# jsnchon/acai-omr

Hardware: AMD Instinct MI355X
Metric: LMX tokens/sec (greedy decode, KV cache) (higher is better)
Workload: dtype bf16; 1 GPU; vitomr_greedy_decode batch 8/GPU of 512x2048 images (4096 patches), decode steps 6..136; batch_per_gpu=8, memory_len=4096, decoder=12 x d1024 h16 mlp4096, V=227, hipgraph=True, split_merge=in-launch

## Files before the change

### acai_omr_amd/_lib.py

```python
import ctypes
import os
import subprocess
from ctypes import POINTER, Structure, c_char_p, c_float, c_int, c_int32, c_int64, c_uint32, c_void_p, c_size_t

CSRC = os.path.join(os.path.dirname(os.path.abspath(__file__)), "csrc")
LIB_PATH = os.environ.get("ACAI_OMR_LIB") or os.path.join(CSRC, "libacai_omr_hip.so")
SOURCES = ["gemm.hip", "elementwise.hip", "attn_varlen.hip", "attn_fwd64.hip", "attn_fwd64w.hip", "attn_bwd.hip", "attn_bwd64w.hip", "attn_bwd1p.hip", "train.hip", "grpo.hip", "seqdist.hip", "decode.hip", "resize.hip"]

ACAI_F32, ACAI_BF16, ACAI_FP8_E4M3 = 0, 1, 2
GEMM_GELU, GEMM_ROUND_BF16 = 1, 2
DEC_CROSS_FP8 = 256


class AcaiDecLayer(Structure):
    _fields_ = [(n, c_void_p) for n in (
        "self_in_w", "self_in_b", "self_out_w", "self_out_b", "cross_q_w", "cross_q_b", "cross_out_w", "cross_out_b",
        "lin1_w", "lin1_b", "lin2_w", "lin2_b", "n1_w", "n1_b", "n2_w", "n2_b", "n3_w", "n3_b",
        "k_self", "v_self", "k_cross", "v_cross", "k_cross_scale", "v_cross_scale")]


class AcaiAdamWTensor(Structure):
    _fields_ = [("p", c_void_p), ("g", c_void_p), ("m", c_void_p), ("v", c_void_p), ("n", c_int64), ("group", c_int32), ("pad_", c_int32),
                ("bias_c1", c_float), ("bias_c2_sqrt", c_float)]

# ... 50 lines not shown
    "acai_attn_varlen_bwd_ws": (c_int, [c_void_p, c_int, c_void_p, c_int, c_void_p, c_int, c_void_p, c_int, c_void_p, c_int, c_void_p, c_int,
                                        c_void_p, c_int, c_void_p, c_int, c_void_p, c_void_p, c_void_p, c_void_p, c_int, c_int, c_int, c_int, c_int,
                                        c_int, c_int, c_int, c_int, c_float, c_uint32, c_int, c_void_p, c_size_t, c_void_p]),
    "acai_attn_varlen_bwd_workspace_bytes": (c_size_t, [c_int, c_int, c_int, c_int, c_int, c_int, c_int, c_int, c_int, c_float, c_int]),
    "acai_dropout_add": (c_int, [c_void_p, c_void_p, c_void_p, c_int, c_int, c_float, c_uint32, c_int, c_int, c_void_p]),
    "acai_layernorm_bwd": (c_int, [c_void_p, c_void_p, c_void_p, c_float, c_void_p, c_void_p, c_void_p, c_void_p, c_void_p, c_void_p, c_int, c_int, c_void_p]),
    "acai_gelu_fwd": (c_int, [c_void_p, c_void_p, c_int64, c_int, c_void_p]),
    "acai_gelu_bwd": (c_int, [c_void_p, c_void_p, c_void_p, c_int64, c_int, c_void_p]),
    "acai_adamw_step": (c_int, [c_void_p, c_void_p, c_void_p, c_void_p, c_int, c_int, c_float, c_void_p]),
    "acai_cast_weights": (c_int, [c_void_p, c_int, c_int, c_void_p]),
    "acai_gemm_dw": (c_int, [c_void_p, c_int, c_void_p, c_int, c_void_p, c_int, c_void_p, c_int, c_int, c_int, c_int, c_void_p]),
    "acai_colsum": (c_int, [c_void_p, c_int, c_void_p, c_int, c_int, c_int, c_void_p]),
    "acai_scatter_add_rows": (c_int, [c_void_p, c_void_p, c_void_p, c_int, c_int, c_int, c_void_p]),
    "acai_mae_loss": (c_int, [c_void_p, c_void_p, c_void_p, c_float, c_void_p, c_void_p, c_int, c_int, c_void_p]),
    "acai_ce_loss": (c_int, [c_void_p, c_int, c_void_p, c_int, c_float, c_float, c_void_p, c_void_p, c_int, c_int, c_void_p]),
    "acai_grpo_objective_fwd": (c_int, [c_void_p, c_int, c_void_p, c_int, c_void_p, c_int, c_void_p, c_void_p, c_int, c_int, c_int, c_float, c_float,
                                        c_int, c_float, c_void_p, c_void_p, c_void_p, c_void_p]),
    "acai_grpo_objective_bwd": (c_int, [c_void_p, c_int, c_void_p, c_int, c_void_p, c_void_p, c_void_p, c_void_p, c_int, c_int, c_int, c_int, c_float,
                                        c_void_p, c_void_p]),
    "acai_edit_distance": (c_int, [c_void_p, c_int, c_void_p, c_void_p, c_int, c_void_p, c_int, c_int, c_void_p, c_void_p]),
    "acai_debug_stamps": (c_int, [c_void_p, c_int]),
    "acai_debug_lds_dma_oob": (c_int, [c_void_p, c_int, c_void_p, c_void_p]),
    "acai_pe_interp_fwd": (c_int, [c_void_p, c_int, c_int, c_int, c_void_p, c_int, c_int, c_void_p]),
    "acai_pe_interp_bwd": (c_int, [c_void_p, c_int, c_int, c_int, c_void_p, c_int, c_int, c_void_p]),
    "acai_cast_f32_bf16": (c_int, [c_void_p, c_void_p, c_int64, c_void_p]),
    "acai_skinny_gemm": (c_int, [c_void_p, c_int, c_void_p, c_int, c_void_p, c_void_p, c_int, c_void_p, c_int, c_int, c_int, c_int,
                                 c_int, c_int, c_void_p]),
    "acai_skinny_gemm_ex": (c_int, [c_void_p, c_int, c_int, c_void_p, c_int, c_void_p, c_void_p, c_int, c_void_p, c_int, c_int, c_int, c_int,
                                    c_int, c_int, c_int, c_void_p, c_void_p, c_float, c_void_p, c_void_p, c_void_p, c_void_p, c_void_p]),
    "acai_decode_attn": (c_int, [c_void_p, c_int, c_void_p, c_void_p, c_void_p, c_void_p, c_void_p, c_void_p, c_int, c_int, c_int,
                                 c_int, c_int, c_int, c_int, c_int, c_int, c_void_p, c_void_p]),
    "acai_decode_attn_fp8": (c_int, [c_void_p, c_int, c_void_p, c_void_p, c_void_p, c_void_p, c_void_p, c_void_p, c_void_p, c_void_p, c_int,
                                     c_int, c_int, c_int, c_int, c_int, c_int, c_int, c_void_p, c_void_p]),
    "acai_cross_kv_quantize_fp8": (c_int, [c_void_p, c_void_p, c_void_p, c_void_p, c_void_p, c_void_p, c_int64, c_int64, c_int, c_void_p]),
    "acai_decode_embed": (c_int, [POINTER(AcaiDecoder), c_void_p]),
    "acai_decode_step": (c_int, [POINTER(AcaiDecoder), c_void_p]),
    "acai_decode_sample_step": (c_int, [POINTER(AcaiDecoder), c_void_p, c_int, c_float, c_void_p]),
    "acai_decode_beam_step": (c_int, [POINTER(AcaiDecoder), POINTER(AcaiBeam), c_void_p]),
    "acai_decode_slot_step": (c_int, [POINTER(AcaiDecoder), POINTER(AcaiSlots), c_void_p]),
    "acai_decode_slot_sample_step": (c_int, [POINTER(AcaiDecoder), POINTER(AcaiSlots), c_void_p, c_int, c_void_p, c_int, c_float,
                                             c_void_p]),
    "acai_decode_slot_arm": (c_int, [POINTER(AcaiDecoder), POINTER(AcaiSlots), c_void_p, c_int, c_void_p]),
    "acai_decode_logits": (c_int, [POINTER(AcaiDecoder), c_void_p, c_int, c_void_p]),
    "acai_decode_hidden": (c_int, [POINTER(AcaiDecoder), c_void_p, c_void_p]),
    "acai_decode_merge_in_launch": (c_int, [c_int, c_int]),
    "acai_graph_begin": (c_int, [c_void_p]),
    "acai_graph_end": (c_int, [c_void_p, POINTER(c_void_p)]),
    "acai_graph_launch": (c_int, [c_void_p, c_void_p]),
    "acai_graph_destroy": (c_int, [c_void_p]),
}

_lib = None


def build(force=False, verbose=False):
    from concurrent.futures import ThreadPoolExecutor
    srcs = [os.path.join(CSRC, s) for s in SOURCES if os.path.exists(os.path.join(CSRC, s))]
    hdrs = sorted(os.path.join(CSRC, f) for f in os.listdir(CSRC) if f.endswith(".h")) + [os.path.join(os.path.dirname(CSRC), "..", "include", "acai_omr_hip.h")]
    hipcc = "hipcc" if subprocess.run(["which", "hipcc"], capture_output=True).returncode == 0 else "/opt/rocm/bin/hipcc"
    flags = ["-O3", "--offload-arch=gfx950", "-std=c++17", "-fPIC", "-Wno-unused-value"]
    per_file = {"attn_varlen.hip": ["-fno-slp-vectorize"], "attn_fwd64.hip": ["-fno-slp-vectorize"],
                "attn_fwd64w.hip": ["-fno-slp-vectorize", "-mllvm", "-amdgpu-mfma-vgpr-form"], "attn_bwd.hip": ["-fno-slp-vectorize"],
                "attn_bwd64w.hip": ["-fno-slp-vectorize", "-mllvm", "-amdgpu-mfma-vgpr-form"],
                "attn_bwd1p.hip": ["-fno-slp-vectorize", "-mllvm", "-amdgpu-mfma-vgpr-form"]}
    objdir = os.path.join(CSRC, "build")
    os.makedirs(objdir, exist_ok=True)
# ... 74 lines not shown
```

### acai_omr_amd/csrc/decode.hip

```cpp
#include <stdlib.h>

#include "common.h"

#include <mutex>
#include <unordered_map>

namespace {

constexpr int SK_KC = 1024;
constexpr int SK_BC = 8;

struct SkinnyArgs {
    const float *x;
    const void *W;
    const float *bias;
    const float *residual;
    float *y;
    int ldx, ldw, ldr, ldy, B, N, K, flags;
    void *k_cache, *v_cache;
    const int32_t *step;
    int E, H, dh, dhp, Tmax;
    const float *ln_w, *ln_b;
    float ln_eps;
    float *stats_out;
// ... 656 lines not shown
    const void *kc, *vc;
    const int64_t *seq_off;
    const int32_t *seq_len;
    const int32_t *step;
    float *partial;
    int ldq, H, dh, dhp, Tmax, chunk, nsplit;
    float scale_log2e;
    float *out;
    int ldo, round_out;
    unsigned *tickets;
    union {
        const int32_t *anc;
        const int32_t *slot_first;
    };
    int anc_pitch;
    long long anc_bstride;
    const float *k_scale, *v_scale;
};

struct fp8e4m3_t {
    uint8_t bits;
};

template <typename TC, int LPK, bool RAGGED, int U = 2, bool ANC = false, bool SLOT = false>
__global__ __launch_bounds__(256) void decode_attn_kernel(DAttnArgs a) {
    static_assert(!(ANC && RAGGED), "the ancestor table indexes the self-attention cache");
    static_assert(!(SLOT && (RAGGED || ANC)), "the ring indexes the self-attention cache of the row itself");
    constexpr bool F8 = sizeof(TC) == 1;
    static_assert(!F8 || RAGGED, "FP8 storage is the cross K/V's only");
    constexpr int EPC = 16 / sizeof(TC), KPW = 64 / LPK;
    __shared__ float red[4][2 + 64];
    const int tid = threadIdx.x, lane = tid & 63, wave = tid >> 6;
    const int kq = lane % LPK, kg = lane / LPK;
    const int split = blockIdx.x, h = blockIdx.y, b = blockIdx.z;
    int len, hstride;
    size_t base;
    if constexpr (RAGGED) {
        len = a.seq_len[b];
        hstride = len * a.dhp;
        base = (size_t)a.seq_off[b] + (size_t)h * hstride;
    } else if constexpr (ANC) {
        len = a.step[1] + 1;
        hstride = a.Tmax * a.dhp;
        base = (size_t)h * hstride;
    } else if constexpr (SLOT) {
        len = a.seq_len[b];
        hstride = a.Tmax * a.dhp;
        base = ((size_t)b * a.H + h) * hstride;
    } else {
        len = a.step[1] + 1;
        hstride = a.Tmax * a.dhp;
        base = ((size_t)b * a.H + h) * hstride;
    }
    float *part = a.partial + (((size_t)b * a.H + h) * a.nsplit + split) * (a.dhp + 2);
    const int c0 = split * a.chunk, c1 = min(len, c0 + a.chunk);
    const bool fused_merge = a.tickets && a.out && a.nsplit > 1;
    if (c0 >= len) {
        if (tid < a.dhp + 2) {
            if (fused_merge) __hip_atomic_store(part + tid, tid == 0 ? -1.0e30f : 0.f, __ATOMIC_RELAXED, __HIP_MEMORY_SCOPE_AGENT);
            else part[tid] = tid == 0 ? -1.0e30f : 0.f;
        }
        if (!fused_merge) return;
        asm volatile("s_waitcnt vmcnt(0)" ::: "memory");
    }
    const TC *Kp = reinterpret_cast<const TC *>(a.kc) + base;
    const TC *Vp = reinterpret_cast<const TC *>(a.vc) + base;
    [[maybe_unused]] const float *Ks = nullptr, *Vs = nullptr;
    if constexpr (F8) {
        const size_t row0 = base >> __builtin_ctz(a.dhp);
        Ks = a.k_scale + row0;
        Vs = a.v_scale + row0;
    }
    [[maybe_unused]] int32_t *anc_s = nullptr;
    if constexpr (ANC) {
        extern __shared__ int32_t anc_dyn[];
        anc_s = anc_dyn;
        const int32_t *ar = a.anc + (size_t)(a.step[0] & 1) * a.anc_bstride + (size_t)b * a.anc_pitch;
        for (int p = c0 + tid; p < c1; p += 256) anc_s[p - c0] = ar[p];
        __syncthreads();
    }
    [[maybe_unused]] int ring0 = 0;
    if constexpr (SLOT) ring0 = a.slot_first[b];
    auto key_off = [&](int key) -> size_t {
        if constexpr (ANC) return (size_t)anc_s[key - c0] * a.H * hstride + (size_t)key * a.dhp;
        else if constexpr (SLOT) {
            const int p = ring0 + key;
            return (size_t)(p >= a.Tmax ? p - a.Tmax : p) * a.dhp;
        } else return (size_t)key * a.dhp;
    };
// ... 96 lines not shown
    }
    float mw = m;
#pragma unroll
    for (int o = LPK; o < 64; o <<= 1) mw = fmaxf(mw, __shfl_xor(mw, o));
    const float f = fast_exp2(m - mw);
    l *= f;
#pragma unroll
    for (int e = 0; e < EPC; ++e) acc[e] *= f;
#pragma unroll
    for (int o = LPK; o < 64; o <<= 1) {
        l += __shfl_xor(l, o);
#pragma unroll
        for (int e = 0; e < EPC; ++e) acc[e] += __shfl_xor(acc[e], o);
    }
    if (kg == 0) {
        if (kq == 0) {
            red[wave][0] = mw;
            red[wave][1] = l;
        }
#pragma unroll
        for (int e = 0; e < EPC; ++e) red[wave][2 + kq * EPC + e] = acc[e];
    }
    __syncthreads();
    if (wave != 0) return;
    const int d = lane;
    const float M = fmaxf(fmaxf(red[0][0], red[1][0]), fmaxf(red[2][0], red[3][0]));
    float v = 0.f, lsum = 0.f;
#pragma unroll
    for (int w = 0; w < 4; ++w) {
        const float f = fast_exp2(red[w][0] - M);
        v += red[w][2 + d] * f;
        lsum += red[w][1] * f;
    }
    if (a.nsplit == 1 && a.out) {
        if (d < a.dh) {
            float o = v / lsum;
            if (a.round_out) o = round_bf16(o);
            a.out[(size_t)b * a.ldo + h * a.dh + d] = o;
        }
        return;
    }
    if (c0 < len && d < a.dhp) {
        if (fused_merge) {
            __hip_atomic_store(part + 2 + d, v, __ATOMIC_RELAXED, __HIP_MEMORY_SCOPE_AGENT);
            if (d == 0) {
                __hip_atomic_store(part, M, __ATOMIC_RELAXED, __HIP_MEMORY_SCOPE_AGENT);
                __hip_atomic_store(part + 1, lsum, __ATOMIC_RELAXED, __HIP_MEMORY_SCOPE_AGENT);
            }
        } else {
            part[2 + d] = v;
            if (d == 0) {
                part[0] = M;
                part[1] = lsum;
            }
        }
    }
    if (!fused_merge) return;
    asm volatile("s_waitcnt vmcnt(0)" ::: "memory");
    int last = 0;
    if (lane == 0) {
        unsigned *cnt = a.tickets + (size_t)b * a.H + h;
        const unsigned t = __hip_atomic_fetch_add(cnt, 1u, __ATOMIC_RELAXED, __HIP_MEMORY_SCOPE_AGENT);
        last = t == (unsigned)(a.nsplit - 1);
        if (last) __hip_atomic_store(cnt, 0u, __ATOMIC_RELAXED, __HIP_MEMORY_SCOPE_AGENT);
    }
    last = __builtin_amdgcn_readfirstlane(last);
    if (!last || d >= a.dhp) return;
    float *p = a.partial + ((size_t)b * a.H + h) * a.nsplit * (a.dhp + 2);
    auto ld = [&](int i) { return __hip_atomic_load(p + i, __ATOMIC_RELAXED, __HIP_MEMORY_SCOPE_AGENT); };
    float Mm = -1.0e30f, lm = 0.f, om = 0.f;
    for (int s0 = 0; s0 < a.nsplit; s0 += 8) {
        float pm[8], pl[8], po[8];
#pragma unroll
        for (int u = 0; u < 8; ++u) {
            const bool in = s0 + u < a.nsplit;
            const int pb = (in ? s0 + u : s0) * (a.dhp + 2);
            pm[u] = in ? ld(pb) : -1.0e30f;
            pl[u] = in ? ld(pb + 1) : 0.f;
            po[u] = in ? ld(pb + 2 + d) : 0.f;
        }
        float Mc = Mm;
#pragma unroll
        for (int u = 0; u < 8; ++u) Mc = fmaxf(Mc, pm[u]);
        const float resc = fast_exp2(Mm - Mc);
        lm *= resc;
        om *= resc;
        Mm = Mc;
#pragma unroll
        for (int u = 0; u < 8; ++u) {
            const float w = fast_exp2(pm[u] - Mm);
            lm += pl[u] * w;
            om += po[u] * w;
        }
    }
    if (d < a.dh) {
        float o = om / lm;
        if (a.round_out) o = round_bf16(o);
        a.out[(size_t)b * a.ldo + h * a.dh + d] = o;
    }
}

__global__ __launch_bounds__(256) void decode_attn_gmfma_kernel(DAttnArgs a, int group, int gtiles) {
    typedef bf16_t TC;
    typedef TileLayout<2, 64> TL;
    constexpr int GT = 16, KT = 32, DHP = 64;
    __shared__ __attribute__((aligned(16))) unsigned char vlds[4][KT * DHP * 2];
    __shared__ float red[4][GT][2 + 64];
    const int tid = threadIdx.x, lane = tid & 63, wave = tid >> 6;
// ... 622 lines not shown
        }
        if (t + 1 < a.Tmax)
            for (int i = lane * 4; i < a.E; i += 256) {
                const float4 ev = *reinterpret_cast<const float4 *>(a.emb + (size_t)tk * a.E + i), pv = *reinterpret_cast<const float4 *>(a.pos + (size_t)(t + 1) * a.E + i);
                *reinterpret_cast<float4 *>(a.x + (size_t)row * a.E + i) = make_float4(ev.x + pv.x, ev.y + pv.y, ev.z + pv.z, ev.w + pv.w);
            }
    }
}

inline int launch_dattn_group(const DAttnArgs &a, int B, int group, hipStream_t st) {
    const int gtm = cdiv(group, 16);
    hipLaunchKernelGGL(decode_attn_gmfma_kernel, dim3(a.nsplit, a.H, (B / group) * gtm), dim3(256), 0, st, a, group, gtm);
    ACAI_LAUNCH_CHECK("decode_attn_gmfma");
    return 0;
}

inline int launch_dattn_fp8(const DAttnArgs &a, int B, hipStream_t st) {
    if (!a.seq_off || !a.k_scale || !a.v_scale) return acai_set_err(-1, "decode_attn: the FP8 cache form needs ragged offsets and K / V scales");
    dim3 grid(a.nsplit, a.H, B);
    switch (a.dhp) {
        case 16: hipLaunchKernelGGL((decode_attn_kernel<fp8e4m3_t, 1, true>), grid, dim3(256), 0, st, a); break;
        case 32: hipLaunchKernelGGL((decode_attn_kernel<fp8e4m3_t, 2, true>), grid, dim3(256), 0, st, a); break;
        case 64: hipLaunchKernelGGL((decode_attn_kernel<fp8e4m3_t, 4, true>), grid, dim3(256), 0, st, a); break;
        default: return acai_set_err(-1, "decode_attn: FP8 cache dhp=%d unsupported (16, 32 or 64)", a.dhp);
    }
    ACAI_LAUNCH_CHECK("decode_attn_fp8");
    return 0;
}

template <typename TC>
int launch_dattn(const DAttnArgs &a, int B, hipStream_t st) {
    const int lpk = a.dhp * (int)sizeof(TC) / 16;
    static const int dattn_u = getenv("ACAI_DATTN_U") ? atoi(getenv("ACAI_DATTN_U")) : 2;
    dim3 grid(a.nsplit, a.H, B);
#define ACAI_DA(L)                                                                                        \
    case L:                                                                                               \
        if (a.seq_off && L == 8 && dattn_u == 4) hipLaunchKernelGGL((decode_attn_kernel<TC, 8, true, 4>), grid, dim3(256), 0, st, a);  \
        else if (a.seq_off && L == 8 && dattn_u == 3) hipLaunchKernelGGL((decode_attn_kernel<TC, 8, true, 3>), grid, dim3(256), 0, st, a);  \
        else if (a.seq_off) hipLaunchKernelGGL((decode_attn_kernel<TC, L, true>), grid, dim3(256), 0, st, a);  \
        else if (a.seq_len) hipLaunchKernelGGL((decode_attn_kernel<TC, L, false, 2, false, true>), grid, dim3(256), 0, st, a);             \
        else if (a.anc) hipLaunchKernelGGL((decode_attn_kernel<TC, L, false, 2, true>), grid, dim3(256), sizeof(int32_t) * a.chunk, st, a); \
        else hipLaunchKernelGGL((decode_attn_kernel<TC, L, false>), grid, dim3(256), 0, st, a);           \
        break;
    switch (lpk) {
        ACAI_DA(1) ACAI_DA(2) ACAI_DA(4) ACAI_DA(8) ACAI_DA(16)
        default: return acai_set_err(-1, "decode_attn: dhp=%d unsupported", a.dhp);
    }
#undef ACAI_DA
    ACAI_LAUNCH_CHECK("decode_attn");
    return 0;
}

template <typename TC>
bool dattn_merge_validated(int dhp) {
    static int cached[5] = {-1, -1, -1, -1, -1};
    static const int force = getenv("ACAI_DATTN_MERGE") ? atoi(getenv("ACAI_DATTN_MERGE")) : -1;
    if (force >= 0) return force != 0;
    const int lpk = dhp * (int)sizeof(TC) / 16;
    int idx = lpk == 1 ? 0 : lpk == 2 ? 1 : lpk == 4 ? 2 : lpk == 8 ? 3 : lpk == 16 ? 4 : -1;
    if (idx < 0) return false;
    if (cached[idx] < 0) {
        auto occ = [](int L, int &n) -> hipError_t {
            switch (L) {
#define ACAI_OCC(LL) case LL: return hipOccupancyMaxActiveBlocksPerMultiprocessor(&n, reinterpret_cast<const void *>(&decode_attn_kernel<TC, LL, true>), 256, 0);
                ACAI_OCC(1) ACAI_OCC(2) ACAI_OCC(4) ACAI_OCC(8) ACAI_OCC(16)
#undef ACAI_OCC
            }
// ... 93 lines not shown
            s.k_cache = kvl->k_self; s.v_cache = kvl->v_self; s.step = d->step;
            s.E = E; s.H = H; s.dh = d->dh; s.dhp = d->dhp; s.Tmax = d->Tmax;
        }
        return launch_skinny<TW>(s, st);
    };
    auto unembed = [&](const float *x, const float *lnw, const float *lnb, float eps, const float *ln2w, const float *ln2b) -> int {
        return skinny(x, E, d->unembed_w, d->unembed_b, nullptr, d->logits, d->V, d->V, E, rnd, nullptr, lnw, lnb, nullptr, nullptr, nullptr,
                      nullptr, eps, ln2w, ln2b);
    };
    const bool cross_f8 = (d->flags & ACAI_DEC_CROSS_FP8) != 0;
    auto attend = [&](const float *q, int ldq, const void *kc, const void *vc, bool cross, const AcaiDecLayer *ly = nullptr) -> int {
        DAttnArgs a{};
        a.q = q; a.kc = kc; a.vc = vc; a.ldq = ldq; a.H = H; a.dh = d->dh; a.dhp = d->dhp; a.Tmax = d->Tmax;
        a.partial = d->partial; a.scale_log2e = sc;
        if (cross && cross_f8) {
            a.seq_off = d->cross_off; a.seq_len = d->cross_len; a.chunk = d->cross_chunk; a.nsplit = d->cross_nsplit;
            a.dhp = d->dhp < 16 ? 16 : d->dhp;
            a.k_scale = ly->k_cross_scale; a.v_scale = ly->v_cross_scale;
            if (a.nsplit == 1 || (d->tickets && dattn_merge_validated_fp8(a.dhp))) {
                a.out = d->attn; a.ldo = E; a.round_out = rnd ? 1 : 0;
                if (a.nsplit > 1) a.tickets = d->tickets;
                return launch_dattn_fp8(a, B, st);
            }
            int r = launch_dattn_fp8(a, B, st);
            if (r) return r;
            hipLaunchKernelGGL(attn_combine_kernel, dim3(H, B), dim3(64), 0, st, d->partial, d->attn, E, H, d->dh, a.dhp, a.nsplit, rnd ? 1 : 0);
            ACAI_LAUNCH_CHECK("attn_combine");
            return 0;
        }
        if (cross) {
            a.seq_off = d->cross_off; a.seq_len = d->cross_len; a.chunk = d->cross_chunk; a.nsplit = d->cross_nsplit;
        } else {
            a.step = d->step; a.chunk = d->self_chunk; a.nsplit = d->self_nsplit;
            if (beam) {
                a.anc = beam->anc; a.anc_pitch = beam->pitch; a.anc_bstride = (long long)beam->rows * beam->pitch;
            }
            if (slots) {
                a.seq_len = slots->t; a.slot_first = slots->first;
            }
        }
        static const bool no_group = getenv("ACAI_DECODE_GROUP_KERNEL") && atoi(getenv("ACAI_DECODE_GROUP_KERNEL")) == 0;
        const int group = (!no_group && sizeof(TW) == 2 && d->dhp == 64 && cross && d->cross_group > 1 && B % d->cross_group == 0) ? d->cross_group : 1;
        if (a.nsplit == 1) {
            a.out = d->attn; a.ldo = E; a.round_out = rnd ? 1 : 0;
            return group > 1 ? launch_dattn_group(a, B, group, st) : launch_dattn<TW>(a, B, st);
        }
        if (d->tickets && (group > 1 || dattn_merge_validated<TW>(d->dhp))) {
            a.out = d->attn; a.ldo = E; a.round_out = rnd ? 1 : 0; a.tickets = d->tickets;
            return group > 1 ? launch_dattn_group(a, B, group, st) : launch_dattn<TW>(a, B, st);
        }
        int r = launch_dattn<TW>(a, B, st);
        if (r) return r;
        hipLaunchKernelGGL(attn_combine_kernel, dim3(H, B), dim3(64), 0, st, d->partial, d->attn, E, H, d->dh, d->dhp, a.nsplit, rnd ? 1 : 0);
        ACAI_LAUNCH_CHECK("attn_combine");
        return 0;
    };

    if (fused) {
        float *st0 = d->stats, *st1 = d->stats + 2 * B, *st2 = d->stats + 4 * B;
        float *zin = d->x, *z1 = d->proj, *z2 = d->xn;
        const float *lnw = nullptr, *lnb = nullptr;
        for (int l = 0; l < d->L; ++l) {
            const AcaiDecLayer *ly = d->layers + l;
            if ((rc = skinny(zin, E, ly->self_in_w, ly->self_in_b, nullptr, d->qkv, 3 * E, 3 * E, E, rnd, ly, lnw, lnb, st0))) return rc;
            if ((rc = attend(d->qkv, 3 * E, ly->k_self, ly->v_self, false))) return rc;
            if ((rc = skinny(d->attn, E, ly->self_out_w, ly->self_out_b, zin, z1, E, E, E, rnd, nullptr, nullptr, nullptr, nullptr, lnw, lnb, st0))) return rc;
// ... 155 lines not shown
    if (tickets && out) {
        a.out = out; a.ldo = ldo; a.round_out = round_out; a.tickets = tickets;
        return dtype == ACAI_BF16 ? launch_dattn<bf16_t>(a, B, st) : launch_dattn<float>(a, B, st);
    }
    int rc = dtype == ACAI_BF16 ? launch_dattn<bf16_t>(a, B, st) : launch_dattn<float>(a, B, st);
    if (rc || !out) return rc;
    hipLaunchKernelGGL(attn_combine_kernel, dim3(H, B), dim3(64), 0, st, partial, out, ldo, H, dh, dhp, nsplit, round_out);
    ACAI_LAUNCH_CHECK("attn_combine");
    return 0;
}

extern "C" int acai_decode_attn_fp8(const float *q, int ldq, const void *kc, const void *vc, const float *k_scale, const float *v_scale,
                                    const int64_t *seq_off, const int32_t *seq_len, float *partial, float *out, int ldo, int B, int H, int dh,
                                    int dhp, int chunk, int nsplit, int round_out, uint32_t *tickets, void *stream) {
    ACAI_CHECK_ARG(q && kc && vc && k_scale && v_scale && seq_off && seq_len && partial, "acai_decode_attn_fp8: null operand");
    ACAI_CHECK_ARG(B > 0 && H > 0 && dh > 0 && dhp >= dh && (dhp == 16 || dhp == 32 || dhp == 64) && chunk > 0 && nsplit > 0,
                   "acai_decode_attn_fp8: bad dims");
    DAttnArgs a{};
    a.q = q; a.kc = kc; a.vc = vc; a.k_scale = k_scale; a.v_scale = v_scale; a.seq_off = seq_off; a.seq_len = seq_len; a.partial = partial;
    a.ldq = ldq; a.H = H; a.dh = dh; a.dhp = dhp; a.chunk = chunk; a.nsplit = nsplit;
    a.scale_log2e = 1.4426950408889634f / sqrtf((float)dh);
    hipStream_t st = (hipStream_t)stream;
    if (tickets && out) {
        a.out = out; a.ldo = ldo; a.round_out = round_out; a.tickets = tickets;
        return launch_dattn_fp8(a, B, st);
    }
    int rc = launch_dattn_fp8(a, B, st);
    if (rc || !out) return rc;
    hipLaunchKernelGGL(attn_combine_kernel, dim3(H, B), dim3(64), 0, st, partial, out, ldo, H, dh, dhp, nsplit, round_out);
    ACAI_LAUNCH_CHECK("attn_combine");
    return 0;
}

extern "C" int acai_debug_stamps(void *buf, int cap_launches) {
    g_stamps = (unsigned long long *)buf;
    g_stamp_cap = buf ? cap_launches : 0;
    g_stamp_next = 0;
    return 0;
}

extern "C" int acai_decode_merge_in_launch(int dtype, int dhp) {
    if (dtype == ACAI_FP8_E4M3) {
        ACAI_CHECK_ARG(dhp == 16 || dhp == 32 || dhp == 64, "acai_decode_merge_in_launch: bad FP8 dhp");
        return dattn_merge_validated_fp8(dhp) ? 1 : 0;
    }
    ACAI_CHECK_ARG((dtype == ACAI_BF16 || dtype == ACAI_F32) && dhp > 0 && dhp <= 64 && (dhp & (dhp - 1)) == 0, "acai_decode_merge_in_launch: bad dtype / dhp");
    return dtype == ACAI_BF16 ? (dattn_merge_validated<bf16_t>(dhp) ? 1 : 0) : (dattn_merge_validated<float>(dhp) ? 1 : 0);
}

extern "C" int acai_decode_hidden(const AcaiDecoder *d, const float *x_in, void *stream) {
    int rc = check_decoder(d);
    if (rc) return rc;
    ACAI_CHECK_ARG(x_in, "acai_decode_hidden: null input");
    hipStream_t st = (hipStream_t)stream;
    hipError_t e = hipMemcpyAsync(d->x, x_in, sizeof(float) * (size_t)d->B * d->E, hipMemcpyDeviceToDevice, st);
    if (e != hipSuccess) return acai_set_err((int)e, "hipMemcpyAsync: %s", hipGetErrorString(e));
    rc = decode(d, nullptr, st, false, false);
    if (rc) return rc;
    hipLaunchKernelGGL(advance_cache_kernel, dim3(1), dim3(1), 0, st, d->step);
    ACAI_LAUNCH_CHECK("advance_cache");
    x_valid_set(d, false);
    return 0;
}

extern "C" int acai_decode_embed(const AcaiDecoder *d, void *stream) {
    int rc = check_decoder(d);
// ... 27 lines not shown
    int rc = check_step(d, "acai_decode_step", chained);
    if (rc) return rc;
    hipStream_t st = (hipStream_t)stream;
    rc = decode(d, nullptr, st, !chained);
    if (rc) return rc;
    hipLaunchKernelGGL(argmax_logprob_kernel, dim3(1), dim3(d->B > 8 ? 1024 : (d->B > 4 ? 512 : 256)), 0, st, d->logits, d->V, d->B, d->seqs, d->logprobs, d->max_len, d->step,
                       d->finished, d->eos, (d->flags & ACAI_GEMM_ROUND_BF16) ? 1 : 0, 1, chained ? (const float *)d->emb : nullptr, (const float *)d->pos, d->x, d->E, d->Tmax);
    ACAI_LAUNCH_CHECK("argmax_logprob");
    return 0;
}

extern "C" int acai_decode_sample_step(const AcaiDecoder *d, const float *uniforms, int top_k, float temperature, void *stream) {
    const bool chained = d && d->E % 4 == 0;
    int rc = check_step(d, "acai_decode_sample_step", chained);
    if (rc) return rc;
    ACAI_CHECK_ARG(uniforms && top_k >= 1 && top_k <= 64 && temperature > 0.f && d->V <= 512,
                   "acai_decode_sample_step: needs uniforms, 1 <= top_k <= 64, temperature > 0, vocabulary <= 512 (top_k=%d V=%d)", top_k, d->V);
    hipStream_t st = (hipStream_t)stream;
    rc = decode(d, nullptr, st, !chained);
    if (rc) return rc;
    hipLaunchKernelGGL(sample_logprob_kernel, dim3(cdiv(d->B, 4)), dim3(256), 0, st, d->logits, d->V, d->B, d->seqs, d->logprobs, d->max_len, d->step,
                       d->finished, d->eos, (d->flags & ACAI_GEMM_ROUND_BF16) ? 1 : 0, uniforms, top_k, 1.0f / temperature,
                       chained ? (const float *)d->emb : nullptr, (const float *)d->pos, d->x, d->E, d->Tmax);
    hipLaunchKernelGGL(sample_bookkeeping_kernel, dim3(1), dim3(64), 0, st, d->B, d->step, d->finished);
    ACAI_LAUNCH_CHECK("sample_logprob");
    return 0;
}

extern "C" int acai_decode_beam_step(const AcaiDecoder *d, const AcaiBeam *bs, void *stream) {
    int rc = check_step(d, "acai_decode_beam_step", true);
    if (rc) return rc;
    ACAI_CHECK_ARG(bs && bs->anc && bs->tok && bs->lp && bs->cum && bs->len, "acai_decode_beam_step: null beam state");
    ACAI_CHECK_ARG(bs->K >= 1 && bs->K <= BEAM_MAX && d->B % bs->K == 0 && bs->rows >= d->B && bs->pitch >= d->max_len && d->V <= 512 &&
                       d->E % 4 == 0 && d->self_chunk <= 16384,
                   "acai_decode_beam_step: needs 1 <= K <= 16 dividing B, rows >= B, pitch >= max_len, vocabulary <= 512, E %% 4 == 0, "
                   "self_chunk <= 16384 (K=%d B=%d rows=%d pitch=%d V=%d E=%d)", bs->K, d->B, bs->rows, bs->pitch, d->V, d->E);
    hipStream_t st = (hipStream_t)stream;
    rc = decode(d, nullptr, st, false, true, bs);
    if (rc) return rc;
    BeamArgs a{};
    a.logits = d->logits; a.V = d->V; a.K = bs->K; a.E = d->E; a.Tmax = d->Tmax; a.pitch = bs->pitch; a.eos = d->eos; a.pad = d->pad;
    a.round_lp = (d->flags & ACAI_GEMM_ROUND_BF16) ? 1 : 0;
    a.step = d->step; a.finished = d->finished; a.emb = d->emb; a.pos = d->pos; a.x = d->x;
    a.anc = bs->anc; a.tok = bs->tok; a.lp = bs->lp; a.bstride = (long long)bs->rows * bs->pitch; a.cum = bs->cum; a.len = bs->len;
    hipLaunchKernelGGL(beam_select_kernel, dim3(d->B / bs->K), dim3(256), 0, st, a);
    ACAI_LAUNCH_CHECK("beam_select");
    hipLaunchKernelGGL(sample_bookkeeping_kernel, dim3(1), dim3(64), 0, st, d->B, d->step, d->finished);
    ACAI_LAUNCH_CHECK("beam_bookkeeping");
    return 0;
}

static int check_slots(const AcaiDecoder *d, const AcaiSlots *sl, const char *fn) {
    int rc = check_unembed(d, fn);
    if (rc) return rc;
    ACAI_CHECK_ARG(d->seqs && d->logprobs && d->finished && d->max_len > 1 && d->max_len <= d->Tmax, "%s: null sequence state or max_len "
                   "outside [2, Tmax] (max_len=%d Tmax=%d)", fn, d->max_len, d->Tmax);
    ACAI_CHECK_ARG(sl && sl->t && sl->first && sl->cap && sl->rows >= d->B, "%s: null slot state or rows < B", fn);
    ACAI_CHECK_ARG(d->cross_group == 1 && d->E % 4 == 0, "%s: needs cross_group == 1 and E %% 4 == 0 (cross_group=%d E=%d)", fn,
                   d->cross_group, d->E);
    return 0;
}

extern "C" int acai_decode_slot_arm(const AcaiDecoder *d, const AcaiSlots *sl, const int32_t *rows, int n, void *stream) {
    int rc = check_slots(d, sl, "acai_decode_slot_arm");
    if (rc) return rc;
    ACAI_CHECK_ARG(n >= 0 && (n == 0 || rows), "acai_decode_slot_arm: bad row list (n=%d)", n);
    if (n > 0) {
// ... 61 lines not shown
```

### acai_omr_amd/engine.py

```python
import contextlib
import ctypes
import os

import weakref

import torch

from . import _lib, ops
from .scheduler import SlotScheduler


class WeightCache:

    def __init__(self):
        self._c = {}

    def __deepcopy__(self, memo):
        return WeightCache()

    def __reduce__(self):
        return (WeightCache, ())

    def invalidate(self):
        self._c.clear()
# ... 111 lines not shown
    ext[:M] = packed
    if fill_row is None:
        ext[M].zero_()
    else:
        ext[M] = fill_row
    idx = torch.full((B, Lm), M, dtype=torch.int32)
    mask = torch.ones(B, Lm, dtype=torch.bool)
    o = 0
    for b, l in enumerate(lens):
        idx[b, :l] = torch.arange(o, o + l, dtype=torch.int32)
        mask[b, :l] = False
        o += l
    out = ops.gather_rows(ext, idx.reshape(-1).to(packed.device))
    return out.view(B, Lm, E), mask.to(packed.device)


def unpad_rows(padded, mask):
    B, Lm, E = padded.shape
    if mask is None:
        return padded.reshape(B * Lm, E).float().contiguous(), [Lm] * B
    lens = (~mask).sum(dim=1).tolist()
    m = mask.cpu()
    for b, l in enumerate(lens):
        if bool(m[b, :l].any()):
            raise ValueError("latent_attention_mask must mark a suffix of each row as padding (as Encoder.create_attention_mask does)")
    idx = torch.cat([torch.arange(b * Lm, b * Lm + l, dtype=torch.int32) for b, l in enumerate(lens)]).to(padded.device)
    return ops.gather_rows(padded.reshape(B * Lm, E).float().contiguous(), idx), lens


class DecodeEngine:

    CROSS_CHUNK = int(os.environ.get("ACAI_CROSS_CHUNK", "1024"))
    CROSS_SLOTS = 512
    CROSS_CHUNK_FP8 = 1024

    @classmethod
    def pick_cross_chunk_fp8(cls, lens, H):
        if "ACAI_CROSS_CHUNK_FP8" in os.environ:
            return int(os.environ["ACAI_CROSS_CHUNK_FP8"])
        return cls.CROSS_CHUNK_FP8

    @classmethod
    def pick_cross_chunk(cls, lens, H):
        if "ACAI_CROSS_CHUNK" in os.environ or not lens:
            return cls.CROSS_CHUNK
        best, best_cost = cls.CROSS_CHUNK, None
        for c in [cls.CROSS_CHUNK] + list(range(512, 4096 + 1, 64)):
            n = sum(-(-l // c) for l in lens) * H
            cost = -(-n // cls.CROSS_SLOTS) * (min(c, max(lens)) + 72)
            if best_cost is None or cost < best_cost:
                best, best_cost = c, cost
        return best

    def __init__(self, blocks, omr, max_batch_size, max_len, prec, device, memory_fp8=False):
        self.blocks = blocks
        self.omr = omr
        self.prec = prec
        self.bf = prec == "bf16"
        self.cdt = torch.bfloat16 if self.bf else torch.float32
        self.device = device
        self.Bmax, self.Tmax = int(max_batch_size), int(max_len)
        self.L = len(blocks.layers)
        self.E = blocks.layers[0].hidden_dim
        self.H = blocks.layers[0].num_heads
        self.dh = self.E // self.H
        es = 2 if self.bf else 4
        dhp = max(16 // es, 1)
        while dhp < self.dh:
            dhp *= 2
        self.dhp = dhp
        self.cross_fp8 = bool(memory_fp8)
        if self.cross_fp8 and not self.bf:
            raise TypeError("an FP8 memory cache needs cache_dtype=torch.bfloat16")
        self.cdhp = max(dhp, 16) if self.cross_fp8 else dhp
        self.k_cross_scale = self.v_cross_scale = None
        self.k_stage = self.v_stage = None
        self.F = blocks.layers[0].linear1.out_features
        self.V = omr.vocab_size if omr is not None else 1
        self.wc = WeightCache()
        z = lambda *s, dt=torch.float32: torch.zeros(*s, dtype=dt, device=device)
        self.k_self = [z(self.Bmax, self.H, self.Tmax, dhp, dt=self.cdt) for _ in range(self.L)]
        self.v_self = [z(self.Bmax, self.H, self.Tmax, dhp, dt=self.cdt) for _ in range(self.L)]
        self.step = z(2, dt=torch.int32)
        self.finished = z(self.Bmax + 1, dt=torch.int32)
        self.seqs = z(self.Bmax, self.Tmax, dt=torch.int64)
        self.logprobs = z(self.Bmax, self.Tmax)
        self.cross_off = z(self.Bmax, dt=torch.int64)
        self.cross_len = z(self.Bmax, dt=torch.int32)
        self.ws = dict(x=z(self.Bmax, self.E), xn=z(self.Bmax, self.E), qkv=z(self.Bmax, 3 * self.E), attn=z(self.Bmax, self.E),
                       proj=z(self.Bmax, self.E), hid=z(self.Bmax, self.F), logits=z(self.Bmax, self.V))
        self.stats = z(6 * self.Bmax)
        self.tickets = z(self.Bmax * self.H, dt=torch.int32)
        self.SELF_CHUNK = self.Tmax
        self.self_nsplit = 1
        self.partial = None
        self.k_cross = self.v_cross = None
        self.cross_cap = 0
        self.graphs = {}
        self.stream = torch.cuda.Stream(device=device)
        self.B = 0
        self.lens = None
        self.group = 1
        self._mode = ("greedy",)
        self.uniforms = None
        self.beam_anc = None
        self._beam_done = 0
        self.slot_t = None
        self.slot_steps = 0
        self.slot_busy = 0
        self.slot_urow = None
        self.slot_uniforms = None
        self.cache_len = 0
        self._desc = None
        self._keep = None

    def prepare(self, mem32, memb, lens, group_size=1):
        G = int(group_size)
        B = len(lens) * G
        self._mode = ("greedy",)
        if B > self.Bmax:
            raise ValueError(f"The current cache has been setup with a max batch size of {self.Bmax}, but found new key tensors with batch size {B}!")
        if G > 1 and self.cross_fp8:
            raise ValueError("an FP8 memory cache does not support grouped cross K/V (group_size > 1: beam search, grouped GRPO rollouts); "
                             "use memory_cache_dtype=None")
        E, H, dhp, dev = self.E, self.H, self.cdhp, self.device
        self._size_cross(sum(lens) * H * dhp, B, lens, G)
        offs, o = [], 0
# ... 490 lines not shown
```

### acai_omr_amd/ops.py

```python
import functools

import math

import torch

from . import _lib
from ._lib import ACAI_BF16, ACAI_F32, GEMM_GELU, GEMM_ROUND_BF16


def _st(t=None):
    return torch.cuda.current_stream(t.device if t is not None else None).cuda_stream


def _on_operand_device(fn):
    @functools.wraps(fn)
    def wrapped(*args, **kw):
        idx = -1
        for a in args:
            if isinstance(a, torch.Tensor) and a.is_cuda:
                if idx < 0:
                    idx = a.device.index
                elif a.device.index != idx:
                    raise RuntimeError(f"{fn.__name__}: operands on different GPUs (cuda:{idx} and {a.device})")
        if idx >= 0 and idx != torch.cuda.current_device():
# ... 263 lines not shown
    out = torch.empty(B, N, dtype=out_dtype, device=x.device)
    flags = (GEMM_GELU if gelu else 0) | (GEMM_ROUND_BF16 if round_bf16 else 0)
    _lib.check(_lib.lib().acai_skinny_gemm_ex(x.data_ptr(), x.stride(0), _dt(x), w.data_ptr(), w.stride(0), _p(bias), _p(residual),
                                              residual.stride(0) if residual is not None else 0, out.data_ptr(), out.stride(0), _dt(out), B, N, K,
                                              _dt(w), flags, _p(ln[0]) if ln else None, _p(ln[1]) if ln else None, float(ln_eps), _p(stats_out),
                                              _p(rln[0]) if rln else None, _p(rln[1]) if rln else None, _p(rstats), _st()), "acai_skinny_gemm_ex")
    return out


def decode_attn(q, kc, vc, seq_off, seq_len, H, dh, dhp, max_len, round_out=False, chunk=256, fused_merge=False, k_scale=None, v_scale=None):
    _chk(q, "q", torch.float32)
    B = q.shape[0]
    nsplit = max(1, -(-int(max_len) // chunk))
    partial = torch.empty(B * H * nsplit * (dhp + 2), dtype=torch.float32, device=q.device)
    out = torch.empty(B, H * dh, dtype=torch.float32, device=q.device)
    tickets = torch.zeros(B * H, dtype=torch.int32, device=q.device) if fused_merge else None
    tk = tickets.data_ptr() if tickets is not None else None
    if kc.dtype == torch.float8_e4m3fn:
        assert vc.dtype == kc.dtype and k_scale is not None and v_scale is not None
        _chk(k_scale, "k_scale", torch.float32), _chk(v_scale, "v_scale", torch.float32)
        _lib.check(_lib.lib().acai_decode_attn_fp8(q.data_ptr(), q.stride(0), kc.data_ptr(), vc.data_ptr(), k_scale.data_ptr(), v_scale.data_ptr(),
                                                   seq_off.data_ptr(), seq_len.data_ptr(), partial.data_ptr(), out.data_ptr(), out.stride(0), B, H,
                                                   dh, dhp, chunk, nsplit, 1 if round_out else 0, tk, _st()), "acai_decode_attn_fp8")
    else:
        assert k_scale is None and v_scale is None, "per-row scales belong to an FP8 cache"
        _lib.check(_lib.lib().acai_decode_attn(q.data_ptr(), q.stride(0), kc.data_ptr(), vc.data_ptr(), seq_off.data_ptr(), seq_len.data_ptr(),
                                               partial.data_ptr(), out.data_ptr(), out.stride(0), B, H, dh, dhp, chunk, nsplit, _dt(kc),
                                               1 if round_out else 0, tk, _st()), "acai_decode_attn")
    if tickets is not None:
        assert int(tickets.abs().sum().item()) == 0, "arrival counters must re-arm to zero"
    return out


_BWD_WS = {}


def _bwd_workspace(device, nbytes):
    key = (device, torch.cuda.current_stream(device).cuda_stream)
    ws = _BWD_WS.get(key)
    if ws is None or ws.numel() < nbytes:
        ws = _BWD_WS[key] = torch.empty(nbytes, dtype=torch.uint8, device=device)
    return ws


def attn_varlen_bwd(q, k, v, o, dout, lse, cu_q, cu_k, H, dh, max_q, max_k, causal, dq, dk, dv, dropout_p=0.0, seed=0, q_prescaled=False, accumulate_dkv=False,
                    lend_workspace=True):
    for t, n in ((q, "q"), (k, "k"), (v, "v"), (o, "o"), (dout, "dout"), (dq, "dq"), (dk, "dk"), (dv, "dv")):
        _chk(t, n)
        assert t.dim() == 2 and t.dtype == q.dtype, n
    _chk(lse, "lse", torch.float32)
    B = cu_q.numel() - 1
    total_q = q.shape[0]
    assert lse.numel() == H * total_q and dout.shape == o.shape
    delta = torch.empty(H * total_q, dtype=torch.float32, device=q.device)
    flags = (1 if causal else 0) | (2 if accumulate_dkv else 0)
    total_k = k.shape[0]
    need = _lib.lib().acai_attn_varlen_bwd_workspace_bytes(B, H, dh, int(max_q), int(max_k), total_q, total_k, flags, _dt(q), float(dropout_p), 1 if q_prescaled else 0)
    ws = _bwd_workspace(q.device, need) if need and lend_workspace else None
    _lib.check(_lib.lib().acai_attn_varlen_bwd_ws(q.data_ptr(), q.stride(0), k.data_ptr(), k.stride(0), v.data_ptr(), v.stride(0), o.data_ptr(), o.stride(0),
                                                  dout.data_ptr(), dout.stride(0), dq.data_ptr(), dq.stride(0), dk.data_ptr(), dk.stride(0), dv.data_ptr(),
                                                  dv.stride(0), lse.data_ptr(), delta.data_ptr(), cu_q.data_ptr(), cu_k.data_ptr(), B, H, dh, int(max_q),
                                                  int(max_k), total_q, total_k, flags, _dt(q), float(dropout_p), int(seed) & 0xFFFFFFFF,
                                                  1 if q_prescaled else 0, _p(ws), need if ws is not None else 0, _st()),
               "acai_attn_varlen_bwd_ws")


# ... 249 lines not shown
```

### include/acai_omr_hip.h

```cpp
#ifndef ACAI_OMR_HIP_H
#define ACAI_OMR_HIP_H

#include <stdint.h>

#ifdef __cplusplus
extern "C" {
#endif

#define ACAI_ABI_VERSION 1
#define ACAI_F32 0
#define ACAI_BF16 1
#define ACAI_FP8_E4M3 2

#define ACAI_GEMM_GELU 1
#define ACAI_GEMM_ROUND_BF16 2

int acai_version(void);
const char *acai_last_error(void);

int acai_layernorm_fwd(const float *x, const float *w, const float *b, float eps, float *out_f32, void *out_bf16,
                       int rows, int dim, void *stream);

int acai_gemm_nt(const void *A, int lda, const void *W, int ldw, const float *bias, const float *residual, int ldr,
                 void *C, int ldc, int M, int N, int K, int in_dtype, int out_dtype, int flags, void *stream);
// ... 145 lines not shown
} AcaiBeam;
int acai_decode_beam_step(const AcaiDecoder *d, const AcaiBeam *bs, void *stream);

typedef struct {
    int32_t *t;
    int32_t *first;
    int32_t *cap;
    int32_t rows;
    int32_t pad_;
} AcaiSlots;
int acai_decode_slot_step(const AcaiDecoder *d, const AcaiSlots *sl, void *stream);
int acai_decode_slot_sample_step(const AcaiDecoder *d, const AcaiSlots *sl, const float *uniforms, int ld_uniforms, const int32_t *urow,
                                 int top_k, float temperature, void *stream);
int acai_decode_slot_arm(const AcaiDecoder *d, const AcaiSlots *sl, const int32_t *rows, int n, void *stream);
int acai_decode_logits(const AcaiDecoder *dec, const int64_t *tokens, int time_step, void *stream);

int acai_decode_hidden(const AcaiDecoder *dec, const float *x_in, void *stream);

int acai_decode_merge_in_launch(int dtype, int dhp);

int acai_skinny_gemm(const float *x, int ldx, const void *W, int ldw, const float *bias, const float *residual, int ldr,
                     float *y, int ldy, int B, int N, int K, int dtype, int flags, void *stream);

int acai_skinny_gemm_ex(const void *x, int ldx, int x_dtype, const void *W, int ldw, const float *bias, const float *residual, int ldr,
                        void *y, int ldy, int y_dtype, int B, int N, int K, int dtype, int flags, const float *ln_w, const float *ln_b,
                        float ln_eps, float *stats_out, const float *rln_w, const float *rln_b, const float *rstats, void *stream);

int acai_decode_attn(const float *q, int ldq, const void *kc, const void *vc, const int64_t *seq_off, const int32_t *seq_len,
                     float *partial, float *out, int ldo, int B, int H, int dh, int dhp, int chunk, int nsplit, int dtype,
                     int round_out, uint32_t *tickets, void *stream);
int acai_decode_attn_fp8(const float *q, int ldq, const void *kc, const void *vc, const float *k_scale, const float *v_scale,
                         const int64_t *seq_off, const int32_t *seq_len, float *partial, float *out, int ldo, int B, int H, int dh,
                         int dhp, int chunk, int nsplit, int round_out, uint32_t *tickets, void *stream);

int acai_cross_kv_quantize_fp8(const void *k_in, const void *v_in, void *k_out, void *v_out, float *k_scale, float *v_scale,
                               int64_t row0, int64_t nrows, int dhp, void *stream);

int acai_graph_begin(void *stream);
int acai_graph_end(void *stream, void **graph_exec_out);
int acai_graph_launch(void *graph_exec, void *stream);
int acai_graph_destroy(void *graph_exec);

#ifdef __cplusplus
}
#endif
#endif
```

Measured before the change: 11740 tokens/s.

## Split decoder self-attention over key chunks with in-launch merge and early exit

Self-attention during decode now splits the KV cache into 384-key chunks instead of one block per (batch, head), with the split index moved to the outermost grid dimension. Blocks whose chunk lies past the current length exit immediately and the ticket merge counts only active splits. This raises parallelism at small batch (8x16 blocks), where long caches left most CUs idle. The cost is extra partial writes, atomic merge traffic and a fallback to a single split when the merge is not validated. A standalone entry point and Python wrapper are added for testing.

```diff
diff --git a/acai_omr_amd/_lib.py b/acai_omr_amd/_lib.py
--- a/acai_omr_amd/_lib.py
+++ b/acai_omr_amd/_lib.py
@@ -106,6 +106,8 @@
                                  c_int, c_int, c_int, c_int, c_int, c_int, c_void_p, c_void_p]),
     "acai_decode_attn_fp8": (c_int, [c_void_p, c_int, c_void_p, c_void_p, c_void_p, c_void_p, c_void_p, c_void_p, c_void_p, c_void_p, c_int,
                                      c_int, c_int, c_int, c_int, c_int, c_int, c_int, c_void_p, c_void_p]),
+    "acai_decode_self_attn": (c_int, [c_void_p, c_int, c_void_p, c_void_p, c_void_p, c_void_p, c_void_p, c_void_p, c_int, c_int64, c_void_p,
+                                      c_void_p, c_int, c_int, c_int, c_int, c_int, c_int, c_int, c_int, c_int, c_int, c_void_p, c_void_p]),
     "acai_cross_kv_quantize_fp8": (c_int, [c_void_p, c_void_p, c_void_p, c_void_p, c_void_p, c_void_p, c_int64, c_int64, c_int, c_void_p]),
     "acai_decode_embed": (c_int, [POINTER(AcaiDecoder), c_void_p]),
     "acai_decode_step": (c_int, [POINTER(AcaiDecoder), c_void_p]),
diff --git a/acai_omr_amd/csrc/decode.hip b/acai_omr_amd/csrc/decode.hip
--- a/acai_omr_amd/csrc/decode.hip
+++ b/acai_omr_amd/csrc/decode.hip
@@ -712,7 +712,7 @@
     __shared__ float red[4][2 + 64];
     const int tid = threadIdx.x, lane = tid & 63, wave = tid >> 6;
     const int kq = lane % LPK, kg = lane / LPK;
-    const int split = blockIdx.x, h = blockIdx.y, b = blockIdx.z;
+    const int split = RAGGED ? blockIdx.x : blockIdx.z, h = RAGGED ? blockIdx.y : blockIdx.x, b = RAGGED ? blockIdx.z : blockIdx.y;
     int len, hstride;
     size_t base;
     if constexpr (RAGGED) {
@@ -735,6 +735,13 @@
     float *part = a.partial + (((size_t)b * a.H + h) * a.nsplit + split) * (a.dhp + 2);
     const int c0 = split * a.chunk, c1 = min(len, c0 + a.chunk);
     const bool fused_merge = a.tickets && a.out && a.nsplit > 1;
+    int n_act = a.nsplit;
+    if constexpr (!RAGGED) {
+        if (fused_merge) {
+            if (c0 >= len) return;
+            n_act = min((len + a.chunk - 1) / a.chunk, a.nsplit);
+        }
+    }
     if (c0 >= len) {
         if (tid < a.dhp + 2) {
             if (fused_merge) __hip_atomic_store(part + tid, tid == 0 ? -1.0e30f : 0.f, __ATOMIC_RELAXED, __HIP_MEMORY_SCOPE_AGENT);
@@ -897,7 +904,7 @@
         v += red[w][2 + d] * f;
         lsum += red[w][1] * f;
     }
-    if (a.nsplit == 1 && a.out) {
+    if (n_act == 1 && a.out) {
         if (d < a.dh) {
             float o = v / lsum;
             if (a.round_out) o = round_bf16(o);
@@ -926,7 +933,7 @@
     if (lane == 0) {
         unsigned *cnt = a.tickets + (size_t)b * a.H + h;
         const unsigned t = __hip_atomic_fetch_add(cnt, 1u, __ATOMIC_RELAXED, __HIP_MEMORY_SCOPE_AGENT);
-        last = t == (unsigned)(a.nsplit - 1);
+        last = t == (unsigned)(n_act - 1);
         if (last) __hip_atomic_store(cnt, 0u, __ATOMIC_RELAXED, __HIP_MEMORY_SCOPE_AGENT);
     }
     last = __builtin_amdgcn_readfirstlane(last);
@@ -934,11 +941,11 @@
     float *p = a.partial + ((size_t)b * a.H + h) * a.nsplit * (a.dhp + 2);
     auto ld = [&](int i) { return __hip_atomic_load(p + i, __ATOMIC_RELAXED, __HIP_MEMORY_SCOPE_AGENT); };
     float Mm = -1.0e30f, lm = 0.f, om = 0.f;
-    for (int s0 = 0; s0 < a.nsplit; s0 += 8) {
+    for (int s0 = 0; s0 < n_act; s0 += 8) {
         float pm[8], pl[8], po[8];
 #pragma unroll
         for (int u = 0; u < 8; ++u) {
-            const bool in = s0 + u < a.nsplit;
+            const bool in = s0 + u < n_act;
             const int pb = (in ? s0 + u : s0) * (a.dhp + 2);
             pm[u] = in ? ld(pb) : -1.0e30f;
             pl[u] = in ? ld(pb + 1) : 0.f;
@@ -1627,7 +1634,7 @@
 int launch_dattn(const DAttnArgs &a, int B, hipStream_t st) {
     const int lpk = a.dhp * (int)sizeof(TC) / 16;
     static const int dattn_u = getenv("ACAI_DATTN_U") ? atoi(getenv("ACAI_DATTN_U")) : 2;
-    dim3 grid(a.nsplit, a.H, B);
+    const dim3 grid = a.seq_off ? dim3(a.nsplit, a.H, B) : dim3(a.H, B, a.nsplit);
 #define ACAI_DA(L)                                                                                        \
     case L:                                                                                               \
         if (a.seq_off && L == 8 && dattn_u == 4) hipLaunchKernelGGL((decode_attn_kernel<TC, 8, true, 4>), grid, dim3(256), 0, st, a);  \
@@ -1787,6 +1794,9 @@
             a.seq_off = d->cross_off; a.seq_len = d->cross_len; a.chunk = d->cross_chunk; a.nsplit = d->cross_nsplit;
         } else {
             a.step = d->step; a.chunk = d->self_chunk; a.nsplit = d->self_nsplit;
+            if (a.nsplit > 1 && !(d->tickets && dattn_merge_validated<TW>(d->dhp))) {
+                a.chunk = d->Tmax; a.nsplit = 1;
+            }
             if (beam) {
                 a.anc = beam->anc; a.anc_pitch = beam->pitch; a.anc_bstride = (long long)beam->rows * beam->pitch;
             }
@@ -2008,6 +2018,30 @@
     return 0;
 }
 
+extern "C" int acai_decode_self_attn(const float *q, int ldq, const void *kc, const void *vc, const int32_t *step, const int32_t *slot_len,
+                                     const int32_t *slot_first, const int32_t *anc, int anc_pitch, long long anc_bstride, float *partial,
+                                     float *out, int ldo, int B, int H, int dh, int dhp, int Tmax, int chunk, int nsplit, int dtype,
+                                     int round_out, uint32_t *tickets, void *stream) {
+    ACAI_CHECK_ARG(q && kc && vc && step && out && (nsplit == 1 || (partial && tickets)), "acai_decode_self_attn: null operand");
+    ACAI_CHECK_ARG(B > 0 && H > 0 && dh > 0 && dhp >= dh && dhp <= 64 && (dhp & (dhp - 1)) == 0 && chunk > 0 && nsplit > 0 && Tmax > 0 &&
+                       (long)chunk * nsplit >= Tmax && (dtype == ACAI_BF16 || dtype == ACAI_F32) && dhp * (dtype == ACAI_BF16 ? 2 : 4) >= 16,
+                   "acai_decode_self_attn: bad dims");
+    ACAI_CHECK_ARG(!(slot_len && anc) && (!slot_len || slot_first) && (!anc || (anc_pitch >= Tmax && chunk <= 16384)),
+                   "acai_decode_self_attn: slot form needs lengths and ring starts, beam form a table of pitch >= Tmax and chunk <= 16384; not both");
+    DAttnArgs a{};
+    a.q = q; a.kc = kc; a.vc = vc; a.step = step; a.partial = partial;
+    a.ldq = ldq; a.H = H; a.dh = dh; a.dhp = dhp; a.Tmax = Tmax; a.chunk = chunk; a.nsplit = nsplit;
+    a.scale_log2e = 1.4426950408889634f / sqrtf((float)dh);
+    a.out = out; a.ldo = ldo; a.round_out = round_out;
+    if (nsplit > 1) a.tickets = tickets;
+    if (slot_len) {
+        a.seq_len = slot_len; a.slot_first = slot_first;
+    } else if (anc) {
+        a.anc = anc; a.anc_pitch = anc_pitch; a.anc_bstride = anc_bstride;
+    }
+    return dtype == ACAI_BF16 ? launch_dattn<bf16_t>(a, B, (hipStream_t)stream) : launch_dattn<float>(a, B, (hipStream_t)stream);
+}
+
 extern "C" int acai_debug_stamps(void *buf, int cap_launches) {
     g_stamps = (unsigned long long *)buf;
     g_stamp_cap = buf ? cap_launches : 0;
@@ -2101,7 +2135,7 @@
     if (rc) return rc;
     ACAI_CHECK_ARG(bs && bs->anc && bs->tok && bs->lp && bs->cum && bs->len, "acai_decode_beam_step: null beam state");
     ACAI_CHECK_ARG(bs->K >= 1 && bs->K <= BEAM_MAX && d->B % bs->K == 0 && bs->rows >= d->B && bs->pitch >= d->max_len && d->V <= 512 &&
-                       d->E % 4 == 0 && d->self_chunk <= 16384,
+                       d->E % 4 == 0 && d->self_chunk <= 16384 && (d->self_nsplit == 1 || d->Tmax <= 16384),
                    "acai_decode_beam_step: needs 1 <= K <= 16 dividing B, rows >= B, pitch >= max_len, vocabulary <= 512, E %% 4 == 0, "
                    "self_chunk <= 16384 (K=%d B=%d rows=%d pitch=%d V=%d E=%d)", bs->K, d->B, bs->rows, bs->pitch, d->V, d->E);
     hipStream_t st = (hipStream_t)stream;
diff --git a/acai_omr_amd/engine.py b/acai_omr_amd/engine.py
--- a/acai_omr_amd/engine.py
+++ b/acai_omr_amd/engine.py
@@ -167,6 +167,7 @@
 
     CROSS_CHUNK = int(os.environ.get("ACAI_CROSS_CHUNK", "1024"))
     CROSS_SLOTS = 512
+    SELF_CHUNK_KEYS = 384
     CROSS_CHUNK_FP8 = 1024
 
     @classmethod
@@ -226,8 +227,9 @@
                        proj=z(self.Bmax, self.E), hid=z(self.Bmax, self.F), logits=z(self.Bmax, self.V))
         self.stats = z(6 * self.Bmax)
         self.tickets = z(self.Bmax * self.H, dt=torch.int32)
-        self.SELF_CHUNK = self.Tmax
-        self.self_nsplit = 1
+        self.SELF_CHUNK = int(os.environ.get("ACAI_SELF_CHUNK", str(self.SELF_CHUNK_KEYS))) or self.Tmax
+        self.SELF_CHUNK = min(self.SELF_CHUNK, self.Tmax)
+        self.self_nsplit = -(-self.Tmax // self.SELF_CHUNK)
         self.partial = None
         self.k_cross = self.v_cross = None
         self.cross_cap = 0
diff --git a/acai_omr_amd/ops.py b/acai_omr_amd/ops.py
--- a/acai_omr_amd/ops.py
+++ b/acai_omr_amd/ops.py
@@ -319,6 +319,27 @@
     return out
 
 
+def decode_self_attn(q, kc, vc, step, H, dh, chunk, round_out=False, slot_len=None, slot_first=None, anc=None):
+    _chk(q, "q", torch.float32), _chk(kc, "kc"), _chk(vc, "vc"), _chk(step, "step", torch.int32)
+    B, (_, _, Tmax, dhp) = q.shape[0], kc.shape
+    assert kc.is_contiguous() and vc.is_contiguous() and kc.shape == vc.shape and kc.shape[1] == H and kc.shape[0] >= B
+    chunk = min(int(chunk), Tmax)
+    nsplit = -(-Tmax // chunk)
+    partial = torch.empty(B * H * nsplit * (dhp + 2), dtype=torch.float32, device=q.device)
+    tickets = torch.zeros(B * H, dtype=torch.int32, device=q.device)
+    out = torch.empty(B, H * dh, dtype=torch.float32, device=q.device)
+    for t in (slot_len, slot_first, anc):
+        if t is not None:
+            _chk(t, "table", torch.int32)
+    _lib.check(_lib.lib().acai_decode_self_attn(q.data_ptr(), q.stride(0), kc.data_ptr(), vc.data_ptr(), step.data_ptr(), _p(slot_len),
+                                                _p(slot_first), _p(anc), anc.shape[2] if anc is not None else 0,
+                                                anc.shape[1] * anc.shape[2] if anc is not None else 0, partial.data_ptr(), out.data_ptr(),
+                                                out.stride(0), B, H, dh, dhp, Tmax, chunk, nsplit, _dt(kc), 1 if round_out else 0,
+                                                tickets.data_ptr(), _st()), "acai_decode_self_attn")
+    assert int(tickets.abs().sum().item()) == 0, "arrival counters must re-arm to zero"
+    return out
+
+
 _BWD_WS = {}
 
 
diff --git a/include/acai_omr_hip.h b/include/acai_omr_hip.h
--- a/include/acai_omr_hip.h
+++ b/include/acai_omr_hip.h
@@ -201,6 +201,10 @@
 int acai_decode_attn_fp8(const float *q, int ldq, const void *kc, const void *vc, const float *k_scale, const float *v_scale,
                          const int64_t *seq_off, const int32_t *seq_len, float *partial, float *out, int ldo, int B, int H, int dh,
                          int dhp, int chunk, int nsplit, int round_out, uint32_t *tickets, void *stream);
+int acai_decode_self_attn(const float *q, int ldq, const void *kc, const void *vc, const int32_t *step, const int32_t *slot_len,
+                          const int32_t *slot_first, const int32_t *anc, int anc_pitch, long long anc_bstride, float *partial,
+                          float *out, int ldo, int B, int H, int dh, int dhp, int Tmax, int chunk, int nsplit, int dtype,
+                          int round_out, uint32_t *tickets, void *stream);
 
 int acai_cross_kv_quantize_fp8(const void *k_in, const void *v_in, void *k_out, void *v_out, float *k_scale, float *v_scale,
                                int64_t row0, int64_t nrows, int dhp, void *stream);
```

Result: slower. 11600 tokens/s (-1.2%).
